# daviddmc/NeSVoR

Hardware: AMD Instinct MI355X
Metric: INR train iters/sec (2^20 samples, L=16 hash, 64-wide MLP) (higher is better)
Workload: dtype f32 (MLP products evaluated on 2-way fp16 splits of the power-of-two-scaled fp32 operands, fp32 accumulation: error against fp64 at or below the fp32 MFMA chain's; the all-fp32-MFMA rate of the same run is in strict_fp32_mfma)

## Files before the change

### nesvor_amd/csrc/mlp.hip

```cpp
#include <hip/hip_runtime.h>
#include <map>
#include <type_traits>
#include <utility>
#include <tuple>
#include <mutex>
#include "common.h"
#include "../../include/nesvor_hip.h"

namespace {

typedef float f32x4 __attribute__((ext_vector_type(4)));

constexpr int kWidth = 64;
constexpr int kHB = kWidth / 16;
#ifndef NESVOR_MLP_G
#define NESVOR_MLP_G 2
#endif
constexpr int kG = NESVOR_MLP_G;
constexpr int kMaxLayers = NESVOR_MAX_MLP_LAYERS;

#ifndef NESVOR_MLP_ABLATE
#define NESVOR_MLP_ABLATE 0
#endif
__device__ __forceinline__ int64_t hgroup(int64_t gi) { return (NESVOR_MLP_ABLATE & 1) ? (gi & 4095) : gi; }
__device__ __forceinline__ int64_t sgroup(int64_t gi) { return (NESVOR_MLP_ABLATE & 2) ? (gi & 4095) : gi; }

struct MlpArgs {
  const float* W[kMaxLayers];
  const float* b[kMaxLayers];
  float* H[kMaxLayers];
  float* dpre[kMaxLayers];
  const float* xa;
  const float* xb;
  float* y;
  float* dxa;
  float* dxb;
  float* dW_partial;
  int64_t N;
  int n_linear;
  int k_a, k_b, b_row0;
  int out_dim;
  int S;
  int total_params;
  int fast;
  int spg_shift;
  int dxa_group;
  int half16;
  int bf16;
  int hi1;
  int off32;
  uint32_t* Hm;
  float* dx_absmax;
  const float* prep;
  float* y_absmax;
  const _Float16* wimg;
};

template <int KB1>
__device__ __forceinline__ void track_absmax(const MlpArgs& a, const f32x4 (&dx)[KB1], float& mx) {
  const int ka_blocks = a.k_a >> 4;
#pragma unroll
  for (int kb = 0; kb < KB1; ++kb)
    if (kb >= ka_blocks) {
#pragma unroll
      for (int r = 0; r < 4; ++r) mx = fmaxf(mx, fabsf(dx[kb][r]));
    }
}
__device__ __forceinline__ void publish_absmax(const MlpArgs& a, float mx) {
  mx = wave_max(mx);
  if ((threadIdx.x & 63) == 0 && mx > 0.f) atomicMax(reinterpret_cast<unsigned int*>(a.dx_absmax), __float_as_uint(mx));
}

__device__ __forceinline__ float relu_f(float x) { return __int_as_float(max(__float_as_int(x), 0)); }

__device__ __forceinline__ f32x4 mfma4(float a, float b, f32x4 c) {
  return __builtin_amdgcn_mfma_f32_16x16x4f32(a, b, c, 0, 0, 0);
}

typedef __bf16 bf16x4 __attribute__((ext_vector_type(4)));
typedef short s16x4 __attribute__((ext_vector_type(4)));
typedef float f32x2 __attribute__((ext_vector_type(2)));
typedef __bf16 bf16x2_t __attribute__((ext_vector_type(2)));
__device__ __forceinline__ s16x4 pack_bf16(const f32x4& v) {
// ... 498 lines not shown
  for (int kb = 0; kb < KB1; ++kb) {
    if (kb < ka_blocks) {
      if (a.dxa != nullptr) {
        if (a.dxa_group) {
          f32x4 sgrp;
#pragma unroll
          for (int r = 0; r < 4; ++r) sgrp[r] = row_sum_dpp(dx[kb][r]);
          if (j == 0) *reinterpret_cast<f32x4*>(a.dxa + (size_t)gi * a.k_a + 16 * kb + 4 * q) = sgrp;
        } else {
          *reinterpret_cast<f32x4*>(a.dxa + (size_t)n * a.k_a + 16 * kb + 4 * q) = dx[kb];
        }
      }
    } else if (a.dxb != nullptr) {
      const int row0 = 16 * (kb - ka_blocks) + 4 * q;
#pragma unroll
      for (int r = 0; r < 4; ++r)
        if (row0 + r < a.k_b) a.dxb[(size_t)(row0 + r) * a.N + n] = dx[kb][r];
    }
  }
}
__device__ __forceinline__ f32x4 load_dy_fast(const MlpArgs& a, int64_t gi, int j, int q) {
  const int64_t n = sgroup(gi) * 16 + j;
  f32x4 g;
#pragma unroll
  for (int r = 0; r < 4; ++r) {
    const float v = a.y[(size_t)min(4 * q + r, a.out_dim - 1) * a.N + n];
    g[r] = 4 * q + r < a.out_dim ? v : 0.f;
  }
  return g;
}

__device__ __forceinline__ void issue_load_b128(f32x4& dst, const float* p) {
  asm volatile("global_load_dwordx4 %0, %1, off" : "=v"(dst) : "v"(p) : "memory");
}
__device__ __forceinline__ void issue_load_b32(float& dst, const float* p) {
  asm volatile("global_load_dword %0, %1, off" : "=v"(dst) : "v"(p) : "memory");
}
__device__ __forceinline__ void issue_load_b64(f32x2& dst, const void* p) {
  asm volatile("global_load_dwordx2 %0, %1, off" : "=v"(dst) : "v"(p) : "memory");
}
__device__ __forceinline__ void issue_load_u16(float& dst, const void* p) {
  asm volatile("global_load_ushort %0, %1, off" : "=v"(dst) : "v"(p) : "memory");
}
__device__ __forceinline__ void pin(f32x2& x) { asm volatile("" : "+v"(x)); }
template <int HT>
__device__ __forceinline__ f32x4 unpack16(const f32x2& v) {
  const uint32_t u0 = __float_as_uint(v[0]), u1 = __float_as_uint(v[1]);
  if constexpr (HT == 2) return f32x4{widen16<2>(u0 & 0xFFFFu), widen16<2>(u0 >> 16), widen16<2>(u1 & 0xFFFFu), widen16<2>(u1 >> 16)};
  else return f32x4{__uint_as_float(u0 << 16), __uint_as_float(u0 & 0xFFFF0000u), __uint_as_float(u1 << 16),
                    __uint_as_float(u1 & 0xFFFF0000u)};
}
__device__ __forceinline__ void await_loads() {
  __builtin_amdgcn_sched_barrier(0);
  asm volatile("s_waitcnt vmcnt(0)" ::: "memory");
}
__device__ __forceinline__ void pin(f32x4& x) { asm volatile("" : "+v"(x)); }
__device__ __forceinline__ void pin(float& x) { asm volatile("" : "+v"(x)); }
template <int IMM> __device__ __forceinline__ void issue_load_b32_s(float& dst, const void* sbase, uint32_t voff) {
  asm volatile("global_load_dword %0, %1, %2 offset:%3" : "=v"(dst) : "v"(voff), "s"(sbase), "i"(IMM) : "memory");
}
template <int IMM> __device__ __forceinline__ void issue_load_b64_s(f32x2& dst, const void* sbase, uint32_t voff) {
  asm volatile("global_load_dwordx2 %0, %1, %2 offset:%3" : "=v"(dst) : "v"(voff), "s"(sbase), "i"(IMM) : "memory");
}
template <int IMM> __device__ __forceinline__ void issue_load_b128_s(f32x4& dst, const void* sbase, uint32_t voff) {
  asm volatile("global_load_dwordx4 %0, %1, %2 offset:%3" : "=v"(dst) : "v"(voff), "s"(sbase), "i"(IMM) : "memory");
}
template <int IMM> __device__ __forceinline__ void issue_load_u16_s(float& dst, const void* sbase, uint32_t voff) {
  asm volatile("global_load_ushort %0, %1, %2 offset:%3" : "=v"(dst) : "v"(voff), "s"(sbase), "i"(IMM) : "memory");
}
template <int IMM> __device__ __forceinline__ void store_b32_s(const void* sbase, uint32_t voff, float v) {
  asm volatile("global_store_dword %0, %1, %2 offset:%3" : : "v"(voff), "v"(v), "s"(sbase), "i"(IMM) : "memory");
}
template <int IMM> __device__ __forceinline__ void store_b32_s_nt(const void* sbase, uint32_t voff, uint32_t v) {
  asm volatile("global_store_dword %0, %1, %2 offset:%3 nt" : : "v"(voff), "v"(v), "s"(sbase), "i"(IMM) : "memory");
}
template <int IMM> __device__ __forceinline__ void store_b128_s_nt(const void* sbase, uint32_t voff, const f32x4& v) {
  asm volatile("global_store_dwordx4 %0, %1, %2 offset:%3 nt\n\ts_nop 1" : : "v"(voff), "v"(v), "s"(sbase), "i"(IMM) : "memory");
}
template <typename F, int... I> __device__ __forceinline__ void static_for_impl(F&& f, std::integer_sequence<int, I...>) {
  (f(std::integral_constant<int, I>{}), ...);
}
template <int N, typename F> __device__ __forceinline__ void static_for(F&& f) { static_for_impl(f, std::make_integer_sequence<int, N>{}); }

#ifndef NESVOR_FWD_MINBLOCKS
#define NESVOR_FWD_MINBLOCKS 2
#endif
template <int KB1, int NH, int SPLM, bool SAVE, bool COMPACT = false, bool OUT1 = false, bool NOB = false>
__global__ __launch_bounds__(256, (SPLM != 0 && KB1 <= 2) ? NESVOR_FWD_MINBLOCKS : 1) void mlp_fwd_pf_kernel(const MlpArgs a) {
  constexpr bool SPL = SPLM != 0;
  static_assert(!NOB || SPLM == 2, "NOB: mode-4 instantiations only");
  extern __shared__ __attribute__((aligned(16))) float lds[];
  const int k_in = a.k_a + a.k_b;
  constexpr int kBlk = 256;
  float* img1 = lds;
  float* imgh = img1 + kHB * KB1 * kBlk;
  float* imgo = imgh + (NH - 1) * kHB * kHB * kBlk;
  float* bias = imgo + 1 * kHB * kBlk;
  float* wout = bias + (NH + 1) * kWidth;
  float unit[NH + 1], inv_unit[NH + 1], mult[NH + 1];
#pragma unroll
  for (int l = 0; l <= NH; ++l) { unit[l] = 1.f; inv_unit[l] = 1.f; mult[l] = 1.f; }
  if constexpr (SPL) {
    const MlpScales sc = mlp_scales(a.prep, NH, a.k_a > 0, false);
#pragma unroll
    for (int l = 0; l <= NH; ++l) {
      unit[l] = uniform_f(sc.sw[l] * sc.sx[l]);
      inv_unit[l] = pow2_inv(unit[l]);
      mult[l] = l == 0 ? sc.sx[0] : uniform_f(sc.sx[l] * inv_unit[l - 1]);
    }
    if (a.wimg != nullptr) {
      copy_image_ct<kHB * KB1 * kBlk, 256>(img1, a.wimg + wimg_offset(NH, KB1, 0));
#pragma unroll
      for (int l = 1; l < NH; ++l) copy_image_ct<kHB * kHB * kBlk, 256>(imgh + (l - 1) * kHB * kHB * kBlk, a.wimg + wimg_offset(NH, KB1, l));
      if constexpr (!OUT1) copy_image_ct<kHB * kBlk, 256>(imgo, a.wimg + wimg_offset(NH, KB1, NH));
    } else {
      build_image_ct<false, SPL, false, kHB, KB1, 256>(img1, a.W[0], kWidth, k_in, sc.sw[0]);
#pragma unroll
      for (int l = 1; l < NH; ++l) build_image_ct<false, SPL, false, kHB, kHB, 256>(imgh + (l - 1) * kHB * kHB * kBlk, a.W[l], kWidth, kWidth, sc.sw[l]);
      if constexpr (!OUT1) build_image_ct<false, SPL, false, 1, kHB, 256>(imgo, a.W[NH], a.out_dim, kWidth, sc.sw[NH]);
    }
  } else {
    build_image_ct<false, SPL, false, kHB, KB1, 256>(img1, a.W[0], kWidth, k_in);
    for (int l = 1; l < NH; ++l) build_image_ct<false, SPL, false, kHB, kHB, 256>(imgh + (l - 1) * kHB * kHB * kBlk, a.W[l], kWidth, kWidth);
    if constexpr (!OUT1) build_image_ct<false, SPL, false, 1, kHB, 256>(imgo, a.W[NH], a.out_dim, kWidth);
  }
  if constexpr (OUT1) {
    for (int e = threadIdx.x; e < kWidth; e += blockDim.x) wout[e] = a.W[NH][e] * inv_unit[NH - 1];
  }
  if constexpr (!NOB) {
    for (int e = threadIdx.x; e < (NH + 1) * kWidth; e += blockDim.x) {
      const int l = e / kWidth, o = e % kWidth;
      float us = 1.f;
#pragma unroll
      for (int t = 0; t <= NH; ++t) us = (t == l && !(OUT1 && t == NH)) ? unit[t] : us;
      bias[e] = (l < NH || o < a.out_dim) ? a.b[l][o] * us : 0.f;
    }
  }
  __syncthreads();

  const int lane = threadIdx.x & 63, wave = __builtin_amdgcn_readfirstlane(threadIdx.x >> 6);
  const int j = lane & 15, q = lane >> 4;
  const int64_t n_tiles = (a.N >> 4) / (4 * kG);
  const int ka_blocks = a.k_a >> 4;
  uint32_t xoff[KB1][4];
#pragma unroll
  for (int kb = 0; kb < KB1; ++kb)
#pragma unroll
    for (int r = 0; r < 4; ++r) {
      const int row = max(min(16 * (kb - ka_blocks) + 4 * q + r, a.k_b - 1), 0);
      xoff[kb][r] = kb < ka_blocks ? (uint32_t)((16 * kb + 4 * q + r) * 4) : (uint32_t)(((int64_t)(a.b_row0 + row) * a.N + j) * 4);
    }
  uint32_t yoff[4];
#pragma unroll
  for (int r = 0; r < 4; ++r) yoff[r] = (uint32_t)(((int64_t)min(4 * q + r, a.out_dim - 1) * a.N + j) * 4);
  const int spg = a.S >> 4;
  auto issue_x = [&](int64_t tile, float (&xr)[kG][KB1][4]) __attribute__((always_inline)) {
    const int64_t g0 = (tile * 4 + wave) * kG;
#pragma unroll
    for (int g = 0; g < kG; ++g) {
      const int64_t gi = g0 + g;
      const int64_t pixel = a.spg_shift >= 0 ? (gi >> a.spg_shift) : gi / spg;
      const char* bbase = reinterpret_cast<const char*>(a.xb) + sgroup(gi) * 64;
      const char* abase = reinterpret_cast<const char*>(a.xa) + pixel * (int64_t)(a.k_a * 4);
#pragma unroll
      for (int kb = 0; kb < KB1; ++kb) {
        const char* base = kb < ka_blocks ? abase : bbase;
#pragma unroll
        for (int r = 0; r < 4; ++r) issue_load_b32_s<0>(xr[g][kb][r], base, xoff[kb][r]);
      }
    }
  };
  auto settle_x = [&](float (&xr)[kG][KB1][4]) __attribute__((always_inline)) {
    await_loads();
#pragma unroll
    for (int g = 0; g < kG; ++g)
#pragma unroll
      for (int kb = 0; kb < KB1; ++kb)
#pragma unroll
        for (int r = 0; r < 4; ++r) pin(xr[g][kb][r]);
  };
  float xr[kG][KB1][4];
#pragma unroll
  for (int g = 0; g < kG; ++g)
#pragma unroll
    for (int kb = 0; kb < KB1; ++kb)
#pragma unroll
      for (int r = 0; r < 4; ++r) xr[g][kb][r] = 0.f;
  float y_mx = 0.f;
  if ((int64_t)blockIdx.x < n_tiles) { issue_x(blockIdx.x, xr); settle_x(xr); }
  for (int64_t tile = blockIdx.x; tile < n_tiles; tile += gridDim.x) {
    const int64_t g0 = (tile * 4 + wave) * kG;
    f32x4 x[kG][KB1];
#pragma unroll
    for (int g = 0; g < kG; ++g)
#pragma unroll
      for (int kb = 0; kb < KB1; ++kb)
#pragma unroll
        for (int r = 0; r < 4; ++r)
          x[g][kb][r] = (kb < ka_blocks || 16 * (kb - ka_blocks) + 4 * q + r < a.k_b) ? xr[g][kb][r] : 0.f;
    issue_x(min(tile + (int64_t)gridDim.x, n_tiles - 1), xr);
    f32x4 h[NH][kG][kHB];
    uint32_t hmask[kG];
#pragma unroll
    for (int g = 0; g < kG; ++g) hmask[g] = 0u;
#pragma unroll
    for (int l = 0; l < NH; ++l) {
#pragma unroll
      for (int ob = 0; ob < kHB; ++ob) {
        const f32x4 bq = NOB ? f32x4{0.f, 0.f, 0.f, 0.f} : *reinterpret_cast<const f32x4*>(bias + l * kWidth + 16 * ob + 4 * q);
#pragma unroll
        for (int g = 0; g < kG; ++g) h[l][g][ob] = bq;
      }
      if (l == 0) apply_layer<KB1, kHB, false, SPLM>(img1, x, h[0], lane, mult[0]);
      else apply_layer<kHB, kHB, false, SPLM>(imgh + (l - 1) * kHB * kHB * kBlk, h[l - 1], h[l], lane, mult[l]);
      if constexpr (SAVE && COMPACT) {
#pragma unroll
        for (int g = 0; g < kG; ++g) {
          uint32_t sg = 0u;
#pragma unroll
          for (int ob = kHB - 1; ob >= 0; --ob)
#pragma unroll
            for (int r = 3; r >= 0; --r) sg = __builtin_amdgcn_alignbit(sg, __float_as_uint(h[l][g][ob][r]), 31);
          hmask[g] = l == 0 ? (~sg & 0xFFFFu) : ((~sg << 16) | hmask[g]);
        }
      }
#pragma unroll
      for (int g = 0; g < kG; ++g)
#pragma unroll
        for (int ob = 0; ob < kHB; ++ob)
#pragma unroll
          for (int r = 0; r < 4; ++r) h[l][g][ob][r] = relu_f(h[l][g][ob][r]);
    }
    f32x4 o[kG][1];
    if constexpr (OUT1) {
      float part[kG];
#pragma unroll
      for (int g = 0; g < kG; ++g) part[g] = 0.f;
#pragma unroll
      for (int ob = 0; ob < kHB; ++ob) {
        const f32x4 w = *reinterpret_cast<const f32x4*>(wout + 16 * ob + 4 * q);
#pragma unroll
        for (int g = 0; g < kG; ++g)
#pragma unroll
          for (int r = 0; r < 4; ++r) part[g] = fmaf(w[r], h[NH - 1][g][ob][r], part[g]);
      }
#pragma unroll
      for (int g = 0; g < kG; ++g) {
        part[g] += __shfl_xor(part[g], 16, 64);
        part[g] += __shfl_xor(part[g], 32, 64);
        o[g][0] = f32x4{NOB ? part[g] : part[g] + bias[NH * kWidth], 0.f, 0.f, 0.f};
      }
    } else {
      const f32x4 bq = NOB ? f32x4{0.f, 0.f, 0.f, 0.f} : *reinterpret_cast<const f32x4*>(bias + NH * kWidth + 4 * q);
#pragma unroll
      for (int g = 0; g < kG; ++g) o[g][0] = bq;
      apply_layer<kHB, 1, false, SPLM>(imgo, h[NH - 1], o, lane, mult[NH]);
      if constexpr (SPL) {
#pragma unroll
        for (int g = 0; g < kG; ++g) o[g][0] *= inv_unit[NH];
      }
    }
    if (a.y_absmax != nullptr) {
#pragma unroll
      for (int g = 0; g < kG; ++g)
#pragma unroll
        for (int r = 0; r < 4; ++r) y_mx = fmaxf(y_mx, fabsf(o[g][0][r]));
    }
    settle_x(xr);
    if constexpr (SAVE && !COMPACT) {
#pragma unroll
      for (int l = 0; l < NH; ++l)
#pragma unroll
        for (int g = 0; g < kG; ++g) {
          const char* hbase = reinterpret_cast<const char*>(a.H[l]) + hgroup(g0 + g) * (int64_t)(kHB * 64 * 16);
          static_for<kHB>([&](auto ob) {
            f32x4 hv = h[l][g][decltype(ob)::value];
            if constexpr (SPL) hv *= inv_unit[l];
            store_b128_s_nt<decltype(ob)::value * 64 * 16>(hbase, (uint32_t)lane * 16u, hv);
          });
        }
    }
    if constexpr (SAVE && COMPACT) {
#pragma unroll
      for (int g = 0; g < kG; ++g)
        store_b32_s_nt<0>(reinterpret_cast<const char*>(a.Hm) + hgroup(g0 + g) * 256, (uint32_t)lane * 4u, hmask[g]);
    }
#pragma unroll
    for (int g = 0; g < kG; ++g) {
      const char* ybase = reinterpret_cast<const char*>(a.y) + sgroup(g0 + g) * 64;
#pragma unroll
      for (int r = 0; r < 4; ++r)
        if (4 * q + r < a.out_dim) store_b32_s<0>(ybase, yoff[r], o[g][0][r]);
    }
  }
  if (a.y_absmax != nullptr) publish_absmax_wg(a.y_absmax, y_mx);
}

template <int KB1, int BF16 = 0>
__global__ __launch_bounds__(256) void mlp_fwd_kernel(const MlpArgs a) {
  extern __shared__ __attribute__((aligned(16))) float lds[];
  const int n_hidden = a.n_linear - 1;
  const int k_in = a.k_a + a.k_b;
  constexpr int kBlk = 256;
  float* img1 = lds;
  float* imgh = img1 + kHB * KB1 * kBlk;
  float* imgo = imgh + (n_hidden - 1) * kHB * kHB * kBlk;
  float* bias = imgo + 1 * kHB * kBlk;
  build_image<BF16>(img1, a.W[0], kWidth, k_in, kHB, KB1);
  for (int l = 1; l < n_hidden; ++l) build_image<BF16>(imgh + (l - 1) * kHB * kHB * kBlk, a.W[l], kWidth, kWidth, kHB, kHB);
  build_image<BF16>(imgo, a.W[n_hidden], a.out_dim, kWidth, 1, kHB);
  for (int e = threadIdx.x; e < a.n_linear * kWidth; e += blockDim.x) {
    const int l = e / kWidth, o = e % kWidth;
    bias[e] = (l < n_hidden || o < a.out_dim) ? a.b[l][o] : 0.f;
  }
  __syncthreads();

  const int lane = threadIdx.x & 63, wave = __builtin_amdgcn_readfirstlane(threadIdx.x >> 6);
  const int j = lane & 15, q = lane >> 4;
  const int64_t n_groups = (a.N + 15) / 16;
  const int64_t n_tiles = (n_groups + 4 * kG - 1) / (4 * kG);
  float y_mx = 0.f;
  for (int64_t tile = blockIdx.x; tile < n_tiles; tile += gridDim.x) {
    const int64_t g0 = (tile * 4 + wave) * kG;
    f32x4 x[kG][KB1];
#pragma unroll
    for (int g = 0; g < kG; ++g) {
      if (a.fast) {
        load_x_fast<KB1>(a, min(g0 + g, n_groups - 1), j, q, x[g]);
      } else {
        const int64_t n = min((g0 + g) * 16 + j, a.N - 1);
#pragma unroll
        for (int kb = 0; kb < KB1; ++kb)
#pragma unroll
          for (int r = 0; r < 4; ++r) x[g][kb][r] = fetch_input(a, 16 * kb + 4 * q + r, n);
      }
    }
    f32x4 h[kG][kHB];
#pragma unroll
    for (int ob = 0; ob < kHB; ++ob) {
// ... 1259 lines not shown
      if (e != hipSuccess) return (int)e;
      raised[fn] = lds;
    }
  }
  if (persistent_tiles > 0) {
    static std::map<std::tuple<int, const void*, size_t>, int> resident;
    static const int fixed = []() { const char* e = getenv("NESVOR_FWD_GRID"); return e ? atoi(e) : 0; }();
    int n_wg = fixed;
    if (n_wg <= 0) {
      int dev = 0;
      if (hipGetDevice(&dev) != hipSuccess) dev = 0;
      std::lock_guard<std::mutex> lock(mu);
      auto it = resident.find(std::make_tuple(dev, fn, lds));
      if (it == resident.end()) {
        int cus = 256, per_cu = 2;
        if (hipDeviceGetAttribute(&cus, hipDeviceAttributeMultiprocessorCount, dev) != hipSuccess) cus = 256;
        if (hipOccupancyMaxActiveBlocksPerMultiprocessor(&per_cu, k, threads, lds) != hipSuccess || per_cu < 1) per_cu = 2;
        if (per_cu > NESVOR_FWD_WGS_PER_CU) per_cu = NESVOR_FWD_WGS_PER_CU;
        it = resident.emplace(std::make_tuple(dev, fn, lds), cus * per_cu).first;
      }
      n_wg = it->second;
    }
    grid = dim3((unsigned)(persistent_tiles < n_wg ? persistent_tiles : n_wg));
  }
  hipLaunchKernelGGL(k, grid, dim3(threads), lds, st, a);
  return (int)hipGetLastError();
}

bool bias_free(const nesvor_mlp_t* d) {
  if (d->weight[0] == nullptr || d->n_hidden < 1 || d->n_hidden + 1 > kMaxLayers) return false;
  for (int l = 0; l <= d->n_hidden; ++l)
    if (d->bias[l] != nullptr) return false;
  return true;
}

int fill_args(MlpArgs* a, const nesvor_mlp_t* d, int64_t N) {
  if (d->width != kWidth || d->n_hidden < 1 || d->n_hidden + 1 > kMaxLayers || d->out_dim < 1 || d->out_dim > 16 ||
      d->k_a < 0 || d->k_b < 0 || d->k_a + d->k_b < 1 || d->k_a + d->k_b > 64 || d->samples_per_pixel < 1)
    return (int)hipErrorInvalidValue;
  a->N = N;
  a->n_linear = d->n_hidden + 1;
  a->k_a = d->k_a; a->k_b = d->k_b; a->b_row0 = d->b_row0; a->out_dim = d->out_dim; a->S = d->samples_per_pixel;
  const bool nob = bias_free(d);
  int n_null = 0;
  for (int l = 0; l < a->n_linear; ++l) n_null += d->bias[l] == nullptr ? 1 : 0;
  if (d->weight[0] != nullptr && n_null != 0 && !(nob && d->bf16_operands == 4)) return (int)hipErrorInvalidValue;
  int total = 0;
  for (int l = 0; l < a->n_linear; ++l) {
    a->W[l] = d->weight[l]; a->b[l] = d->bias[l];
    const int in = l == 0 ? d->k_a + d->k_b : kWidth, out = l == d->n_hidden ? d->out_dim : kWidth;
    total += in * out + (nob ? 0 : out);
  }
  for (int l = a->n_linear; l < kMaxLayers; ++l) { a->W[l] = nullptr; a->b[l] = nullptr; }
  a->total_params = total;
  const int S = d->samples_per_pixel;
  a->fast = (N % 16 == 0 && S % 16 == 0 && d->k_a % 16 == 0) ? 1 : 0;
  a->dxa_group = d->dxa_group_sums ? 1 : 0;
  a->bf16 = d->bf16_operands;
  if (a->bf16 < 0 || a->bf16 > 4) return (int)hipErrorInvalidValue;
  a->hi1 = 0;
  if (a->bf16 == 4) { a->bf16 = 2; a->hi1 = 1; }
  a->half16 = a->bf16 == 3 ? 1 : 0;
  if (a->half16) a->bf16 = 1;
  a->prep = d->prep;
  a->y_absmax = d->y_absmax;
  a->wimg = (a->bf16 == 2) ? static_cast<const _Float16*>(d->weight_images) : nullptr;
  {
    const int64_t rows = (int64_t)(d->b_row0 + d->k_b > d->out_dim ? d->b_row0 + d->k_b : d->out_dim);
    a->off32 = rows * N * 4 + 64 < ((int64_t)1 << 32) ? 1 : 0;
  }
  a->spg_shift = -1;
  if (a->fast) {
    const int spg = S / 16;
    if ((spg & (spg - 1)) == 0) a->spg_shift = __builtin_ctz(spg);
  }
  return 0;
}

bool out1_on() {
  static const bool on = []() { const char* e = getenv("NESVOR_MLP_OUT1"); return e == nullptr || atoi(e) != 0; }();
  return on;
}

bool compact_ok(const MlpArgs& a, const nesvor_mlp_t* net, int64_t N) {
  static const bool use_pf = []() { const char* e = getenv("NESVOR_MLP_FWD_PF"); return e == nullptr || atoi(e) != 0; }();
  static const bool use_ws = []() { const char* e = getenv("NESVOR_MLP_BWD_WS"); return e == nullptr || atoi(e) != 0; }();
  static const bool on = []() { const char* e = getenv("NESVOR_MLP_COMPACT"); return e == nullptr || atoi(e) != 0; }();
  const int kb1 = (net->k_a + net->k_b + 15) / 16;
  return on && use_pf && use_ws && a.bf16 == 2 && a.fast && a.off32 && net->n_hidden <= 2 && kb1 <= 2 && ((N >> 4) % (4 * kG)) == 0;
}

bool ws_ok(const MlpArgs& a, const nesvor_mlp_t* net) {
  static const bool use_ws = []() { const char* e = getenv("NESVOR_MLP_BWD_WS"); return e == nullptr || atoi(e) != 0; }();
  const int kb1 = (net->k_a + net->k_b + 15) / 16;
  return use_ws && a.fast && a.off32 && net->n_hidden <= 2 && (kb1 <= 2 || net->n_hidden == 1);
}

}

#if NESVOR_MLP_TIMELINE
extern "C" int nesvor_debug_mlp_timeline(unsigned long long* dst_host) {
  return (int)hipMemcpyFromSymbol(dst_host, HIP_SYMBOL(g_mlp_timeline), sizeof(unsigned long long) * 64 * 8 * 4);
}
#endif

extern "C" int nesvor_mlp_backward_fused_ok(const nesvor_mlp_t* net, int64_t N) {
  if (net == nullptr || N <= 0) return 0;
  MlpArgs a{};
  if (fill_args(&a, net, N)) return 0;
  if (bias_free(net)) return compact_ok(a, net, N) ? 1 : 0;
  return ws_ok(a, net) ? 1 : 0;
}

extern "C" int nesvor_mlp_bias_free_ok(const nesvor_mlp_t* net, int64_t N) {
  if (net == nullptr || N <= 0 || net->weight[0] == nullptr) return 0;
  nesvor_mlp_t d = *net;
  for (int l = 0; l < kMaxLayers; ++l) d.bias[l] = nullptr;
  MlpArgs a{};
  if (fill_args(&a, &d, N) || !bias_free(&d)) return 0;
  for (int l = 0; l <= d.n_hidden; ++l)
    if (d.weight[l] == nullptr) return 0;
  return d.k_b >= 1 ? 1 : 0;
}

extern "C" int64_t nesvor_mlp_weight_images_bytes(const nesvor_mlp_t* net) {
  if (net == nullptr || net->n_hidden < 1 || net->n_hidden + 1 > kMaxLayers || net->width != kWidth || net->k_a + net->k_b < 1 ||
      net->k_a + net->k_b > 64 || net->out_dim < 1 || net->out_dim > 16)
    return 0;
  const int kb1 = (net->k_a + net->k_b + 15) / 16;
  return (int64_t)sizeof(_Float16) * wimg_offset(net->n_hidden, kb1, net->n_hidden + 1);
}

extern "C" int nesvor_mlp_prepare_weights_images(const nesvor_mlp_t* const* nets, float* const* preps, void* const* images, int n_nets,
                                                 const float* x, int64_t n_x, float* x_slots, void* stream) {
  if (n_nets < 0 || n_nets > 3 || (n_nets > 0 && (nets == nullptr || preps == nullptr))) return (int)hipErrorInvalidValue;
  NormJobs jobs{};
  int nj = 0;
  for (int i = 0; i < n_nets; ++i) {
    const nesvor_mlp_t* net = nets[i];
    if (net == nullptr || preps[i] == nullptr || net->n_hidden < 1 || net->n_hidden + 1 > kMaxLayers || net->width != kWidth ||
        net->k_a + net->k_b > 64 || net->out_dim > 64)
      return (int)hipErrorInvalidValue;
    _Float16* img = (images != nullptr && net->out_dim <= 16) ? static_cast<_Float16*>(images[i]) : nullptr;
    const int kb1 = (net->k_a + net->k_b + 15) / 16;
    for (int l = 0; l <= net->n_hidden; ++l, ++nj) {
      jobs.W[nj] = net->weight[l]; jobs.b[nj] = net->bias[l];
      jobs.in[nj] = l == 0 ? net->k_a + net->k_b : net->width;
      jobs.out[nj] = l == net->n_hidden ? net->out_dim : net->width;
      jobs.dst[nj] = preps[i] + NESVOR_MLP_PREP_LAYER0 + 4 * l;
      jobs.img[nj] = img != nullptr ? img + wimg_offset(net->n_hidden, kb1, l) : nullptr;
      jobs.oblk[nj] = l == net->n_hidden ? 1 : kHB;
      jobs.iblk[nj] = l == 0 ? kb1 : kHB;
      if (jobs.W[nj] == nullptr) return (int)hipErrorInvalidValue;
    }
  }
  jobs.n_jobs = nj;
  const bool with_x = x != nullptr && x_slots != nullptr && n_x > 0;
  jobs.x = x; jobs.n_x = with_x ? n_x : 0; jobs.x_slots = x_slots;
  if (nj + (with_x ? 1 : 0) == 0) return 0;
  hipLaunchKernelGGL(weight_norms_kernel, dim3((unsigned)(nj + (with_x ? 1 : 0))), dim3(256), 0, (hipStream_t)stream, jobs);
  return (int)hipGetLastError();
}

extern "C" int nesvor_mlp_prepare_weights(const nesvor_mlp_t* const* nets, float* const* preps, int n_nets, const float* x, int64_t n_x,
                                          float* x_slots, void* stream) {
  return nesvor_mlp_prepare_weights_images(nets, preps, nullptr, n_nets, x, n_x, x_slots, stream);
// ... 16 lines not shown
    if (e) return e;
    e = absmax(xb != nullptr ? xb + (size_t)net->b_row0 * N : nullptr, net->k_b, N, N, prep + NESVOR_MLP_PREP_XB);
    if (e) return e;
  }
  if (what & NESVOR_MLP_WHAT_DY) {
    const int e = absmax(dy, net->out_dim, N, N, prep + NESVOR_MLP_PREP_DY);
    if (e) return e;
  }
  if (what & NESVOR_MLP_WHAT_WEIGHTS) return nesvor_mlp_prepare_weights(&net, &prep, 1, nullptr, 0, nullptr, stream);
  return (int)hipGetLastError();
}

extern "C" int nesvor_mlp_compact_save_ok(const nesvor_mlp_t* net, int64_t N) {
  if (net == nullptr || N <= 0) return 0;
  MlpArgs a{};
  if (fill_args(&a, net, N)) return 0;
  return compact_ok(a, net, N) ? 1 : 0;
}

extern "C" int nesvor_mlp_forward(const nesvor_mlp_t* net, const float* xa, const float* xb, float* y,
                                  float* const* saved_hidden, int64_t N, void* stream) {
  if (N <= 0) return 0;
  MlpArgs a{};
  int e = fill_args(&a, net, N);
  if (e) return e;
  a.xa = xa; a.xb = xb; a.y = y;
  for (int l = 0; l < kMaxLayers; ++l) a.H[l] = (saved_hidden != nullptr && l < net->n_hidden) ? saved_hidden[l] : nullptr;
  const int kb1 = (net->k_a + net->k_b + 15) / 16;
  const int64_t n_tiles = ((N + 15) / 16 + 4 * kG - 1) / (4 * kG);
  dim3 grid((unsigned)(n_tiles < 512 ? n_tiles : 512));
  static const bool use_pf = []() { const char* e = getenv("NESVOR_MLP_FWD_PF"); return e == nullptr || atoi(e) != 0; }();
  bool save_all = saved_hidden != nullptr, save_none = saved_hidden == nullptr;
  const bool compact = net->compact_save != 0 && save_all;
  if (a.bf16 == 2 && a.prep == nullptr) return (int)hipErrorInvalidValue;
  if (bias_free(net)) {
    const size_t lds = fwd_lds_bytes(a.n_linear, kb1);
    const bool pf = use_pf && a.fast && a.off32 && net->n_hidden <= 2 && kb1 <= 2 && ((N >> 4) % (4 * kG)) == 0;
    if (compact) {
      if (!compact_ok(a, net, N)) return (int)hipErrorInvalidValue;
      a.Hm = reinterpret_cast<uint32_t*>(saved_hidden[0]);
      a.H[0] = nullptr;
      if (net->out_dim == 1 && out1_on()) {
        if (net->n_hidden == 1)
          return launch_kb(mlp_fwd_pf_kernel<1, 1, 2, true, true, true, true>, mlp_fwd_pf_kernel<2, 1, 2, true, true, true, true>,
                           mlp_fwd_pf_kernel<2, 1, 2, true, true, true, true>, mlp_fwd_pf_kernel<2, 1, 2, true, true, true, true>, kb1, grid,
                           lds, (hipStream_t)stream, a, 256, n_tiles);
        return launch_kb(mlp_fwd_pf_kernel<1, 2, 2, true, true, true, true>, mlp_fwd_pf_kernel<2, 2, 2, true, true, true, true>,
                         mlp_fwd_pf_kernel<2, 2, 2, true, true, true, true>, mlp_fwd_pf_kernel<2, 2, 2, true, true, true, true>, kb1, grid,
                         lds, (hipStream_t)stream, a, 256, n_tiles);
      }
      if (net->n_hidden == 1)
        return launch_kb(mlp_fwd_pf_kernel<1, 1, 2, true, true, false, true>, mlp_fwd_pf_kernel<2, 1, 2, true, true, false, true>,
                         mlp_fwd_pf_kernel<2, 1, 2, true, true, false, true>, mlp_fwd_pf_kernel<2, 1, 2, true, true, false, true>, kb1, grid,
                         lds, (hipStream_t)stream, a, 256, n_tiles);
      return launch_kb(mlp_fwd_pf_kernel<1, 2, 2, true, true, false, true>, mlp_fwd_pf_kernel<2, 2, 2, true, true, false, true>,
                       mlp_fwd_pf_kernel<2, 2, 2, true, true, false, true>, mlp_fwd_pf_kernel<2, 2, 2, true, true, false, true>, kb1, grid,
                       lds, (hipStream_t)stream, a, 256, n_tiles);
    }
    if (pf && save_none) {
      if (net->n_hidden == 1)
        return launch_kb(mlp_fwd_pf_kernel<1, 1, 2, false, false, false, true>, mlp_fwd_pf_kernel<2, 1, 2, false, false, false, true>,
                         mlp_fwd_pf_kernel<2, 1, 2, false, false, false, true>, mlp_fwd_pf_kernel<2, 1, 2, false, false, false, true>, kb1,
                         grid, lds, (hipStream_t)stream, a, 256, n_tiles);
      return launch_kb(mlp_fwd_pf_kernel<1, 2, 2, false, false, false, true>, mlp_fwd_pf_kernel<2, 2, 2, false, false, false, true>,
                       mlp_fwd_pf_kernel<2, 2, 2, false, false, false, true>, mlp_fwd_pf_kernel<2, 2, 2, false, false, false, true>, kb1,
                       grid, lds, (hipStream_t)stream, a, 256, n_tiles);
    }
    nesvor_mlp_wide_t w{};
    w.width = kWidth; w.n_hidden = net->n_hidden; w.out_dim = net->out_dim; w.k_a = net->k_a; w.k_b = net->k_b; w.b_row0 = net->b_row0;
    w.samples_per_pixel = net->samples_per_pixel;
    for (int l = 0; l <= net->n_hidden; ++l) { w.weight[l] = net->weight[l]; w.bias[l] = nullptr; }
    e = nesvor_mlp_wide_forward(&w, xa, xb, y, save_all ? saved_hidden : nullptr, N, stream);
    if (e || a.y_absmax == nullptr) return e;
    const int64_t work = ((int64_t)net->out_dim * N + 1023) / 1024;
    hipLaunchKernelGGL(absmax_rows_kernel, dim3((unsigned)(work < 2048 ? (work < 1 ? 1 : work) : 2048)), dim3(256), 0, (hipStream_t)stream, y,
                       net->out_dim, N, N, a.y_absmax);
    return (int)hipGetLastError();
  }
  if (compact) {
    if (!compact_ok(a, net, N)) return (int)hipErrorInvalidValue;
    a.Hm = reinterpret_cast<uint32_t*>(saved_hidden[0]);
    a.H[0] = nullptr;
    const size_t lds = fwd_lds_bytes(a.n_linear, kb1);
    if (a.hi1) {
      if (net->out_dim == 1 && out1_on()) {
        if (net->n_hidden == 1)
          return launch_kb(mlp_fwd_pf_kernel<1, 1, 2, true, true, true>, mlp_fwd_pf_kernel<2, 1, 2, true, true, true>,
                           mlp_fwd_pf_kernel<2, 1, 2, true, true, true>, mlp_fwd_pf_kernel<2, 1, 2, true, true, true>, kb1, grid, lds,
                           (hipStream_t)stream, a, 256, n_tiles);
        return launch_kb(mlp_fwd_pf_kernel<1, 2, 2, true, true, true>, mlp_fwd_pf_kernel<2, 2, 2, true, true, true>,
                         mlp_fwd_pf_kernel<2, 2, 2, true, true, true>, mlp_fwd_pf_kernel<2, 2, 2, true, true, true>, kb1, grid, lds,
                         (hipStream_t)stream, a, 256, n_tiles);
      }
      if (net->n_hidden == 1)
        return launch_kb(mlp_fwd_pf_kernel<1, 1, 2, true, true>, mlp_fwd_pf_kernel<2, 1, 2, true, true>, mlp_fwd_pf_kernel<2, 1, 2, true, true>,
                         mlp_fwd_pf_kernel<2, 1, 2, true, true>, kb1, grid, lds, (hipStream_t)stream, a, 256, n_tiles);
      return launch_kb(mlp_fwd_pf_kernel<1, 2, 2, true, true>, mlp_fwd_pf_kernel<2, 2, 2, true, true>, mlp_fwd_pf_kernel<2, 2, 2, true, true>,
                       mlp_fwd_pf_kernel<2, 2, 2, true, true>, kb1, grid, lds, (hipStream_t)stream, a, 256, n_tiles);
    }
    if (net->out_dim == 1 && out1_on()) {
      if (net->n_hidden == 1)
        return launch_kb(mlp_fwd_pf_kernel<1, 1, true, true, true, true>, mlp_fwd_pf_kernel<2, 1, true, true, true, true>,
                         mlp_fwd_pf_kernel<2, 1, true, true, true, true>, mlp_fwd_pf_kernel<2, 1, true, true, true, true>, kb1, grid, lds,
                         (hipStream_t)stream, a, 256, n_tiles);
      return launch_kb(mlp_fwd_pf_kernel<1, 2, true, true, true, true>, mlp_fwd_pf_kernel<2, 2, true, true, true, true>,
                       mlp_fwd_pf_kernel<2, 2, true, true, true, true>, mlp_fwd_pf_kernel<2, 2, true, true, true, true>, kb1, grid, lds,
                       (hipStream_t)stream, a, 256, n_tiles);
    }
    if (net->n_hidden == 1)
      return launch_kb(mlp_fwd_pf_kernel<1, 1, true, true, true>, mlp_fwd_pf_kernel<2, 1, true, true, true>, mlp_fwd_pf_kernel<2, 1, true, true, true>,
                       mlp_fwd_pf_kernel<2, 1, true, true, true>, kb1, grid, lds, (hipStream_t)stream, a, 256, n_tiles);
    return launch_kb(mlp_fwd_pf_kernel<1, 2, true, true, true>, mlp_fwd_pf_kernel<2, 2, true, true, true>, mlp_fwd_pf_kernel<2, 2, true, true, true>,
                     mlp_fwd_pf_kernel<2, 2, true, true, true>, kb1, grid, lds, (hipStream_t)stream, a, 256, n_tiles);
  }
  if (use_pf && a.bf16 != 1 && a.fast && a.off32 && net->n_hidden <= 2 && ((N >> 4) % (4 * kG)) == 0 && (save_all || save_none)) {
    const bool x6 = a.bf16 == 2;
    const size_t lds = fwd_lds_bytes(a.n_linear, kb1);
    if (x6 && a.hi1 && save_none && kb1 <= 2) {
      if (net->n_hidden == 1)
        return launch_kb(mlp_fwd_pf_kernel<1, 1, 2, false>, mlp_fwd_pf_kernel<2, 1, 2, false>, mlp_fwd_pf_kernel<2, 1, 2, false>,
                         mlp_fwd_pf_kernel<2, 1, 2, false>, kb1, grid, lds, (hipStream_t)stream, a, 256, n_tiles);
      return launch_kb(mlp_fwd_pf_kernel<1, 2, 2, false>, mlp_fwd_pf_kernel<2, 2, 2, false>, mlp_fwd_pf_kernel<2, 2, 2, false>,
                       mlp_fwd_pf_kernel<2, 2, 2, false>, kb1, grid, lds, (hipStream_t)stream, a, 256, n_tiles);
    }
#define NESVOR_PF(NH, SPL, SAVE) launch_kb(mlp_fwd_pf_kernel<1, NH, SPL, SAVE>, mlp_fwd_pf_kernel<2, NH, SPL, SAVE>, \
      mlp_fwd_pf_kernel<3, NH, SPL, SAVE>, mlp_fwd_pf_kernel<4, NH, SPL, SAVE>, kb1, grid, lds, (hipStream_t)stream, a, 256, n_tiles)
    if (net->n_hidden == 1) {
      if (x6) return save_all ? NESVOR_PF(1, true, true) : NESVOR_PF(1, true, false);
      return save_all ? NESVOR_PF(1, false, true) : NESVOR_PF(1, false, false);
    }
    if (x6) return save_all ? NESVOR_PF(2, true, true) : NESVOR_PF(2, true, false);
    return save_all ? NESVOR_PF(2, false, true) : NESVOR_PF(2, false, false);
#undef NESVOR_PF
  }
  if (a.bf16 == 1 && a.half16)
    return launch_kb(mlp_fwd_kernel<1, 2>, mlp_fwd_kernel<2, 2>, mlp_fwd_kernel<3, 2>, mlp_fwd_kernel<4, 2>, kb1,
                     grid, fwd_lds_bytes(a.n_linear, kb1), (hipStream_t)stream, a);
  if (a.bf16 == 1)
    return launch_kb(mlp_fwd_kernel<1, true>, mlp_fwd_kernel<2, true>, mlp_fwd_kernel<3, true>, mlp_fwd_kernel<4, true>, kb1,
                     grid, fwd_lds_bytes(a.n_linear, kb1), (hipStream_t)stream, a);
  return launch_kb(mlp_fwd_kernel<1>, mlp_fwd_kernel<2>, mlp_fwd_kernel<3>, mlp_fwd_kernel<4>, kb1, grid,
                   fwd_lds_bytes(a.n_linear, kb1), (hipStream_t)stream, a);
}

extern "C" int nesvor_mlp_backward(const nesvor_mlp_t* net, const float* xa, const float* xb, const float* dy,
                                   float* const* saved_hidden, float* const* dpre_scratch, float* dxa, float* dxb,
                                   float* dw_partial, int n_partial, int64_t N, void* stream) {
  return nesvor_mlp_backward_bounded(net, xa, xb, dy, saved_hidden, dpre_scratch, dxa, dxb, dw_partial, n_partial, N, nullptr, stream);
}

extern "C" int nesvor_mlp_backward_bounded(const nesvor_mlp_t* net, const float* xa, const float* xb, const float* dy,
                                           float* const* saved_hidden, float* const* dpre_scratch, float* dxa, float* dxb,
                                           float* dw_partial, int n_partial, int64_t N, float* dxb_absmax, void* stream) {
  if (N <= 0) return 0;
  MlpArgs a{};
  int e = fill_args(&a, net, N);
  if (e) return e;
  a.dx_absmax = dxb != nullptr ? dxb_absmax : nullptr;
  if (saved_hidden == nullptr || dpre_scratch == nullptr || dw_partial == nullptr || n_partial < 1) return (int)hipErrorInvalidValue;
  const bool split = a.bf16 == 2;
  const bool compact = net->compact_save != 0;
  if (split && a.prep == nullptr) return (int)hipErrorInvalidValue;
  if (compact && (!compact_ok(a, net, N) || dpre_scratch[0] != nullptr)) return (int)hipErrorInvalidValue;
  if (split) a.bf16 = 0;
  a.xa = xa; a.xb = xb; a.y = const_cast<float*>(dy); a.dxa = dxa; a.dxb = dxb; a.dW_partial = dw_partial;
  for (int l = 0; l < kMaxLayers; ++l) {
// ... 126 lines not shown
```

Before: 1058.

## Interleave MLP forward layer epilogues with next group's MFMAs in compact-save kernel

Adds an interleaved schedule to the compact-save split-mode forward MLP kernel. Each layer's epilogue work for one sample group (sign-mask build, ReLU, fp16 hi/lo splitting via mixed FMA) is spread between the MFMA issues of the other group, with weight fragments double-buffered from LDS one block pair ahead. It targets the serial gap between matrix ops and vector epilogue work and is on by default for two hidden layers with kb1==2. The cost is higher register pressure and hand-placed scheduling barriers, which could hurt occupancy or block compiler scheduling.

```diff
diff --git a/nesvor_amd/csrc/mlp.hip b/nesvor_amd/csrc/mlp.hip
--- a/nesvor_amd/csrc/mlp.hip
+++ b/nesvor_amd/csrc/mlp.hip
@@ -1,4 +1,5 @@
 #include <hip/hip_runtime.h>
+#include <cstring>
 #include <map>
 #include <type_traits>
 #include <utility>
@@ -663,13 +664,98 @@
 }
 template <int N, typename F> __device__ __forceinline__ void static_for(F&& f) { static_for_impl(f, std::make_integer_sequence<int, N>{}); }
 
+struct SplitRegs { uint32_t h0, h1, l0, l1; };
+template <int U>
+__device__ __forceinline__ void split2_unit(const f32x4& v, float m, SplitRegs& r) {
+  if constexpr (U == 0) {
+    asm volatile("v_fma_mixlo_f16 %0, %1, %2, 0" : "=v"(r.h0) : "v"(v[0]), "s"(m));
+    asm volatile("v_fma_mixlo_f16 %0, %1, %2, 0" : "=v"(r.h1) : "v"(v[2]), "s"(m));
+  } else if constexpr (U == 1) {
+    asm volatile("v_fma_mixhi_f16 %0, %1, %2, 0" : "+v"(r.h0) : "v"(v[1]), "s"(m));
+    asm volatile("v_fma_mixhi_f16 %0, %1, %2, 0" : "+v"(r.h1) : "v"(v[3]), "s"(m));
+  } else if constexpr (U == 2) {
+    asm volatile("v_fma_mixlo_f16 %0, %1, %2, -%3 op_sel:[0,0,0] op_sel_hi:[0,0,1]" : "=v"(r.l0) : "v"(v[0]), "s"(m), "v"(r.h0));
+    asm volatile("v_fma_mixlo_f16 %0, %1, %2, -%3 op_sel:[0,0,0] op_sel_hi:[0,0,1]" : "=v"(r.l1) : "v"(v[2]), "s"(m), "v"(r.h1));
+  } else {
+    asm volatile("v_fma_mixhi_f16 %0, %1, %2, -%3 op_sel:[0,0,1] op_sel_hi:[0,0,1]" : "+v"(r.l0) : "v"(v[1]), "s"(m), "v"(r.h0));
+    asm volatile("v_fma_mixhi_f16 %0, %1, %2, -%3 op_sel:[0,0,1] op_sel_hi:[0,0,1]" : "+v"(r.l1) : "v"(v[3]), "s"(m), "v"(r.h1));
+  }
+}
+__device__ __forceinline__ f16x8 join8u(uint32_t a, uint32_t b, uint32_t c, uint32_t d) {
+  asm("" : "+v"(a)); asm("" : "+v"(b)); asm("" : "+v"(c)); asm("" : "+v"(d));
+  const f32x4 v{__uint_as_float(a), __uint_as_float(b), __uint_as_float(c), __uint_as_float(d)};
+  return __builtin_bit_cast(f16x8, v);
+}
+constexpr int ilv_pairs(int kb1, int l) { return l == 0 ? kb1 / 2 : kHB / 2; }
+constexpr int ilv_block0(int kb1, int s) {
+  int i = 0;
+  for (int t = 0; t < s; ++t) i += ilv_pairs(kb1, t / kG);
+  return i;
+}
+constexpr int ilv_phase_of(int kb1, int i) {
+  int s = 0;
+  while (ilv_block0(kb1, s + 1) <= i) ++s;
+  return s;
+}
+template <int KB, int OB, int PLANE, int P, int NW>
+__device__ __forceinline__ void load_frags_ilv(const float* __restrict__ img, int lane, f16x8 (&w)[NW]) {
+  const _Float16* img16 = reinterpret_cast<const _Float16*>(img) + PLANE * (OB * KB * 256);
+  constexpr int kb = 2 * P;
+#pragma unroll
+  for (int ob = 0; ob < OB; ++ob)
+    w[ob] = join8h(*reinterpret_cast<const s16x4*>(img16 + ((ob * KB + kb) * 64 + lane) * 4),
+                   *reinterpret_cast<const s16x4*>(img16 + ((ob * KB + kb + 1) * 64 + lane) * 4));
+}
+template <int KB, bool HI1, int J0, typename Fill, typename Next>
+__device__ __forceinline__ void apply_layer_ilv(f16x8 (&wf)[2][kHB], const SplitRegs (&b)[kHB], f32x4 (&y)[kHB], Fill&& fill, Next&& next) {
+  static_assert(KB % 2 == 0, "whole pairs of input blocks");
+  constexpr int T = HI1 ? 1 : 3;
+  static_for<KB / 2>([&](auto pc) __attribute__((always_inline)) {
+    constexpr int p = decltype(pc)::value, kb = 2 * p, j = J0 + p;
+    const f16x8 bh = join8u(b[kb].h0, b[kb].h1, b[kb + 1].h0, b[kb + 1].h1);
+    f16x8 bl = bh;
+    if constexpr (!HI1) bl = join8u(b[kb].l0, b[kb].l1, b[kb + 1].l0, b[kb + 1].l1);
+    static_for<T>([&](auto tc) __attribute__((always_inline)) {
+      constexpr int t = decltype(tc)::value;
+      if constexpr (HI1) next(std::integral_constant<int, j + 1>{}, std::integral_constant<int, 0>{}, wf[(j + 1) & 1]);
+      else if constexpr (t == 0) next(std::integral_constant<int, j>{}, std::integral_constant<int, 0>{}, wf[0]);
+      else if constexpr (t == 1) next(std::integral_constant<int, j + 1>{}, std::integral_constant<int, 1>{}, wf[1]);
+      static_for<kHB>([&](auto oc) __attribute__((always_inline)) {
+        constexpr int ob = decltype(oc)::value;
+        y[ob] = mfma32_f16(wf[HI1 ? (j & 1) : (t == 0 ? 1 : 0)][ob], (!HI1 && t == 1) ? bl : bh, y[ob]);
+        __builtin_amdgcn_sched_barrier(0);
+        fill(std::integral_constant<int, (p * T + t) * kHB + ob>{});
+        __builtin_amdgcn_sched_barrier(0);
+      });
+    });
+  });
+}
+template <bool HI1, typename Fill>
+__device__ __forceinline__ void apply_out_ilv(const f16x8 (&wo)[kHB / 2][2], const SplitRegs (&b)[kHB], f32x4& y, Fill&& fill) {
+  constexpr int T = HI1 ? 1 : 3;
+  static_for<kHB / 2>([&](auto pc) __attribute__((always_inline)) {
+    constexpr int p = decltype(pc)::value, kb = 2 * p;
+    const f16x8 bh = join8u(b[kb].h0, b[kb].h1, b[kb + 1].h0, b[kb + 1].h1);
+    f16x8 bl = bh;
+    if constexpr (!HI1) bl = join8u(b[kb].l0, b[kb].l1, b[kb + 1].l0, b[kb + 1].l1);
+    static_for<T>([&](auto tc) __attribute__((always_inline)) {
+      constexpr int t = decltype(tc)::value;
+      y = mfma32_f16(wo[p][(!HI1 && t == 0) ? 1 : 0], (!HI1 && t == 1) ? bl : bh, y);
+      __builtin_amdgcn_sched_barrier(0);
+      fill(std::integral_constant<int, p * T + t>{});
+      __builtin_amdgcn_sched_barrier(0);
+    });
+  });
+}
+
 #ifndef NESVOR_FWD_MINBLOCKS
 #define NESVOR_FWD_MINBLOCKS 2
 #endif
-template <int KB1, int NH, int SPLM, bool SAVE, bool COMPACT = false, bool OUT1 = false, bool NOB = false>
+template <int KB1, int NH, int SPLM, bool SAVE, bool COMPACT = false, bool OUT1 = false, bool NOB = false, bool ILV = false>
 __global__ __launch_bounds__(256, (SPLM != 0 && KB1 <= 2) ? NESVOR_FWD_MINBLOCKS : 1) void mlp_fwd_pf_kernel(const MlpArgs a) {
   constexpr bool SPL = SPLM != 0;
   static_assert(!NOB || SPLM == 2, "NOB: mode-4 instantiations only");
+  static_assert(!ILV || (SPL && SAVE && COMPACT && KB1 % 2 == 0 && kG == 2), "ILV: compact-save split-mode instantiations, whole block pairs, two groups");
   extern __shared__ __attribute__((aligned(16))) float lds[];
   const int k_in = a.k_a + a.k_b;
   constexpr int kBlk = 256;
@@ -769,6 +855,28 @@
       for (int r = 0; r < 4; ++r) xr[g][kb][r] = 0.f;
   float y_mx = 0.f;
   if ((int64_t)blockIdx.x < n_tiles) { issue_x(blockIdx.x, xr); settle_x(xr); }
+  f16x8 wf[2][kHB], wo[kHB / 2][2];
+  constexpr int kIlvBlocks = ilv_block0(KB1 - KB1 % 2, kG * NH);
+  auto ilv_next = [&](auto jc, auto planec, f16x8 (&dst)[kHB]) __attribute__((always_inline)) {
+    constexpr int j = decltype(jc)::value % kIlvBlocks, s = ilv_phase_of(KB1, j), l = s / kG, pr = j - ilv_block0(KB1, s);
+    if constexpr (l == 0) load_frags_ilv<KB1, kHB, decltype(planec)::value, pr>(img1, lane, dst);
+    else load_frags_ilv<kHB, kHB, decltype(planec)::value, pr>(imgh + (l - 1) * kHB * kHB * kBlk, lane, dst);
+  };
+  if constexpr (ILV) {
+    static_assert(kIlvBlocks % 2 == 0, "mode 4: the register set of a block must not change from tile to tile");
+    if constexpr (SPLM == 2) ilv_next(std::integral_constant<int, 0>{}, std::integral_constant<int, 0>{}, wf[0]);
+    else ilv_next(std::integral_constant<int, 0>{}, std::integral_constant<int, 1>{}, wf[1]);
+    if constexpr (!OUT1) {
+      static_for<kHB / 2>([&](auto pc) __attribute__((always_inline)) {
+        f16x8 t0[1], t1[1];
+        load_frags_ilv<kHB, 1, 0, decltype(pc)::value>(imgo, lane, t0);
+        if constexpr (SPLM != 2) load_frags_ilv<kHB, 1, 1, decltype(pc)::value>(imgo, lane, t1);
+        else t1[0] = t0[0];
+        wo[decltype(pc)::value][0] = t0[0];
+        wo[decltype(pc)::value][1] = t1[0];
+      });
+    }
+  }
   for (int64_t tile = blockIdx.x; tile < n_tiles; tile += gridDim.x) {
     const int64_t g0 = (tile * 4 + wave) * kG;
     f32x4 x[kG][KB1];
@@ -784,8 +892,76 @@
     uint32_t hmask[kG];
 #pragma unroll
     for (int g = 0; g < kG; ++g) hmask[g] = 0u;
-#pragma unroll
-    for (int l = 0; l < NH; ++l) {
+    f32x4 o[kG][1];
+    if constexpr (ILV) {
+      constexpr bool HI1 = SPLM == 2;
+      constexpr int SU = HI1 ? 2 : 4;
+      constexpr int LM = OUT1 ? NH : NH + 1;
+      SplitRegs bsr[kG][kHB];
+      uint32_t sg[kG];
+      constexpr auto epi_units = [](int l) { return l < 0 ? KB1 * SU + (HI1 ? 1 : 0) : 8 + kHB * (2 + ((OUT1 && l == NH - 1) ? 0 : SU)); };
+      auto epi = [&](auto lc, auto gc, auto uc) __attribute__((always_inline)) {
+        constexpr int l = decltype(lc)::value, g = decltype(gc)::value, u = decltype(uc)::value;
+        if constexpr (l < 0) {
+          if constexpr (u < KB1 * SU) split2_unit<u % SU>(x[g][u / SU], mult[0], bsr[g][u / SU]);
+          else asm("s_nop 1" : "+v"(bsr[g][0].h0), "+v"(bsr[g][0].h1), "+v"(bsr[g][KB1 - 1].h0), "+v"(bsr[g][KB1 - 1].h1));
+        } else if constexpr (u < 8) {
+          if constexpr (u == 0) sg[g] = 0u;
+          constexpr int i0 = 15 - 2 * u, i1 = 14 - 2 * u;
+          sg[g] = __builtin_amdgcn_alignbit(sg[g], __float_as_uint(h[l][g][i0 / 4][i0 % 4]), 31);
+          sg[g] = __builtin_amdgcn_alignbit(sg[g], __float_as_uint(h[l][g][i1 / 4][i1 % 4]), 31);
+          if constexpr (u == 7) hmask[g] = l == 0 ? (~sg[g] & 0xFFFFu) : ((~sg[g] << 16) | hmask[g]);
+        } else {
+          constexpr bool SPLIT = !(OUT1 && l == NH - 1);
+          constexpr int PER = 2 + (SPLIT ? SU : 0), ob = (u - 8) / PER, w = (u - 8) % PER;
+          if constexpr (w < 2) {
+            h[l][g][ob][2 * w] = relu_f(h[l][g][ob][2 * w]);
+            h[l][g][ob][2 * w + 1] = relu_f(h[l][g][ob][2 * w + 1]);
+          } else {
+            split2_unit<w - 2>(h[l][g][ob], mult[l < NH ? l + 1 : NH], bsr[g][ob]);
+          }
+        }
+      };
+      auto init_acc = [&](auto sc) __attribute__((always_inline)) {
+        constexpr int s = decltype(sc)::value, l = s / kG, g = s % kG;
+        if constexpr (l < NH) {
+#pragma unroll
+          for (int ob = 0; ob < kHB; ++ob)
+            h[l][g][ob] = NOB ? f32x4{0.f, 0.f, 0.f, 0.f} : *reinterpret_cast<const f32x4*>(bias + l * kWidth + 16 * ob + 4 * q);
+        } else if constexpr (l < LM) {
+          o[g][0] = NOB ? f32x4{0.f, 0.f, 0.f, 0.f} : *reinterpret_cast<const f32x4*>(bias + NH * kWidth + 4 * q);
+        }
+      };
+      init_acc(std::integral_constant<int, 0>{});
+      static_for<epi_units(-1)>([&](auto uc) __attribute__((always_inline)) { epi(std::integral_constant<int, -1>{}, std::integral_constant<int, 0>{}, uc); });
+      static_for<kG * LM>([&](auto sc) __attribute__((always_inline)) {
+        constexpr int s = decltype(sc)::value, l = s / kG, g = s % kG;
+        constexpr int el = (s + 1) / kG - 1, eg = (s + 1) % kG;
+        constexpr int KB = l == 0 ? KB1 : kHB, OB = l == NH ? 1 : kHB, NM = KB / 2 * (HI1 ? 1 : 3) * OB;
+        static_assert(NM > 0);
+        constexpr int U = el < NH ? epi_units(el) : 0;
+        auto fill = [&](auto mc) __attribute__((always_inline)) {
+          constexpr int m = decltype(mc)::value, u0 = U * m / NM, u1 = U * (m + 1) / NM;
+          static_for<u1 - u0>([&](auto uc) __attribute__((always_inline)) {
+            epi(std::integral_constant<int, el>{}, std::integral_constant<int, eg>{}, std::integral_constant<int, u0 + decltype(uc)::value>{});
+          });
+        };
+        init_acc(std::integral_constant<int, s + 1>{});
+        if constexpr (l < NH) {
+          static_assert(ilv_block0(KB1, s + 1) - ilv_block0(KB1, s) == KB / 2);
+          apply_layer_ilv<KB, HI1, ilv_block0(KB1, s)>(wf, bsr[g], h[l][g], fill, ilv_next);
+        } else {
+          apply_out_ilv<HI1>(wo, bsr[g], o[g][0], fill);
+        }
+      });
+      if constexpr (OUT1) {
+        static_for<epi_units(NH - 1)>([&](auto uc) __attribute__((always_inline)) {
+          epi(std::integral_constant<int, NH - 1>{}, std::integral_constant<int, kG - 1>{}, uc);
+        });
+      }
+    }
+#pragma unroll
+    for (int l = 0; l < (ILV ? 0 : NH); ++l) {
 #pragma unroll
       for (int ob = 0; ob < kHB; ++ob) {
         const f32x4 bq = NOB ? f32x4{0.f, 0.f, 0.f, 0.f} : *reinterpret_cast<const f32x4*>(bias + l * kWidth + 16 * ob + 4 * q);
@@ -812,7 +988,6 @@
 #pragma unroll
           for (int r = 0; r < 4; ++r) h[l][g][ob][r] = relu_f(h[l][g][ob][r]);
     }
-    f32x4 o[kG][1];
     if constexpr (OUT1) {
       float part[kG];
 #pragma unroll
@@ -833,9 +1008,11 @@
       }
     } else {
       const f32x4 bq = NOB ? f32x4{0.f, 0.f, 0.f, 0.f} : *reinterpret_cast<const f32x4*>(bias + NH * kWidth + 4 * q);
-#pragma unroll
-      for (int g = 0; g < kG; ++g) o[g][0] = bq;
-      apply_layer<kHB, 1, false, SPLM>(imgo, h[NH - 1], o, lane, mult[NH]);
+      if constexpr (!ILV) {
+#pragma unroll
+        for (int g = 0; g < kG; ++g) o[g][0] = bq;
+        apply_layer<kHB, 1, false, SPLM>(imgo, h[NH - 1], o, lane, mult[NH]);
+      }
       if constexpr (SPL) {
 #pragma unroll
         for (int g = 0; g < kG; ++g) o[g][0] *= inv_unit[NH];
@@ -2261,6 +2438,11 @@
   return on;
 }
 
+bool mlp_sched_interleaved() {
+  static const bool on = []() { const char* e = getenv("NESVOR_MLP_SCHED"); return e == nullptr || strcmp(e, "block") != 0; }();
+  return on;
+}
+
 bool compact_ok(const MlpArgs& a, const nesvor_mlp_t* net, int64_t N) {
   static const bool use_pf = []() { const char* e = getenv("NESVOR_MLP_FWD_PF"); return e == nullptr || atoi(e) != 0; }();
   static const bool use_ws = []() { const char* e = getenv("NESVOR_MLP_BWD_WS"); return e == nullptr || atoi(e) != 0; }();
@@ -2443,6 +2625,17 @@
     a.Hm = reinterpret_cast<uint32_t*>(saved_hidden[0]);
     a.H[0] = nullptr;
     const size_t lds = fwd_lds_bytes(a.n_linear, kb1);
+    const bool ilv = mlp_sched_interleaved() && net->n_hidden == 2 && kb1 == 2;
+#define NESVOR_PF_ILV(SPLM, OUT1)                                                                                            \
+  launch_kb(mlp_fwd_pf_kernel<2, 2, SPLM, true, true, OUT1, false, true>, mlp_fwd_pf_kernel<2, 2, SPLM, true, true, OUT1, false, true>, \
+            mlp_fwd_pf_kernel<2, 2, SPLM, true, true, OUT1, false, true>, mlp_fwd_pf_kernel<2, 2, SPLM, true, true, OUT1, false, true>, \
+            kb1, grid, lds, (hipStream_t)stream, a, 256, n_tiles)
+    if (ilv) {
+      const bool out1 = net->out_dim == 1 && out1_on();
+      if (a.hi1) return out1 ? NESVOR_PF_ILV(2, true) : NESVOR_PF_ILV(2, false);
+      return out1 ? NESVOR_PF_ILV(1, true) : NESVOR_PF_ILV(1, false);
+    }
+#undef NESVOR_PF_ILV
     if (a.hi1) {
       if (net->out_dim == 1 && out1_on()) {
         if (net->n_hidden == 1)
```

Measured after the change: 1055. Within noise of the previous version (-0.4%).
